# oneapi-src/ishmem

Hardware: AMD Instinct MI355X
Metric: GiB/s device-resident float32 sum-reduce at 1/2/4/8 PEs vs HBM+xGMI roofline (higher is better)
Workload: dtype f32

## Files before the change

include/ishmem_capi.h:

```cpp
#ifndef ISHMEM_AMD_CAPI_H
#define ISHMEM_AMD_CAPI_H

#include <stddef.h>
#include <stdint.h>

#ifdef __cplusplus
extern "C" {
#endif

typedef enum {
    ISHMEMI_OP_AND = 0,
    ISHMEMI_OP_OR = 1,
    ISHMEMI_OP_XOR = 2,
    ISHMEMI_OP_MAX = 3,
    ISHMEMI_OP_MIN = 4,
    ISHMEMI_OP_SUM = 5,
    ISHMEMI_OP_PROD = 6,
    ISHMEMI_OP_COUNT = 7
} ishmemi_c_op_t;

typedef enum {
    ISHMEMI_DT_INT8 = 0,
    ISHMEMI_DT_INT16 = 1,
    ISHMEMI_DT_INT32 = 2,
// ... 137 lines not shown
#define ISHMEMI_C_AMO_COUNT 14
int ishmemi_c_amo(int op, int dtype, void *dest, uint64_t value_bits, uint64_t cond_bits, int pe, uint64_t *fetched_bits);
int ishmemi_c_amo_nbi(int op, int dtype, void *fetch, void *dest, uint64_t value_bits, uint64_t cond_bits, int pe);

#define ISHMEMI_C_MAX_PES 16
#define ISHMEMI_C_MAX_TEAMS 64
#define ISHMEMI_C_DEV_PHASES 4
typedef struct {
    int32_t pe, npes;
    uint64_t timeout_ticks;
    char *heap_base;
    uint64_t heap_size;
    char *peer_heap[ISHMEMI_C_MAX_PES];
    uint32_t *my_dflags;
    uint32_t *peer_dflags[ISHMEMI_C_MAX_PES];
    uint32_t *epochs;
    uint32_t *err;
    int32_t team_start[ISHMEMI_C_MAX_TEAMS], team_stride[ISHMEMI_C_MAX_TEAMS];
    int32_t team_size[ISHMEMI_C_MAX_TEAMS], team_my_idx[ISHMEMI_C_MAX_TEAMS];
    uint64_t *dev_counts;
} ishmemi_c_device_ctx_t;
void *ishmemi_c_device_ctx(void);
int ishmemi_c_register_device_ctx_slot(const void *host_shadow);

const char *ishmemi_c_last_error(void);
int ishmemi_c_set_param(const char *name, long long value);
long long ishmemi_c_get_param(const char *name);
int ishmemi_c_phase_times(float *ms5);
int ishmemi_c_error_count(void);
size_t ishmemi_c_dtype_size(int dtype);
int ishmemi_c_op_dtype_valid(int op, int dtype);
int ishmemi_c_chunk_bounds(uint64_t nitems, int npes, int c, uint64_t *begin, uint64_t *end);
int ishmemi_c_path_limits(int npes, int colocated, long long *ll_limit, long long *fold_limit);
int ishmemi_c_bootstrap_selftest(int pe, int npes, const char *key, int value, int *out);
const char *ishmemi_c_version(void);

#ifdef __cplusplus
}
#endif

#endif
```

ishmem_amd/_lib.py:

```python
from __future__ import annotations

import ctypes
import os
from pathlib import Path

LIB_PATH = Path(__file__).resolve().parent / "libishmem_amd.so"
_VARIANT = os.environ.get("ISHMEM_AMD_LIB")

_vp, _i, _sz, _ll, _u64 = ctypes.c_void_p, ctypes.c_int, ctypes.c_size_t, ctypes.c_longlong, ctypes.c_uint64
PROTOTYPES = [
    ("ishmemi_c_init", _i, []),
    ("ishmemi_c_init_pe", _i, [_i, _i, _i, ctypes.c_char_p]),
    ("ishmemi_c_launch_info", _i, [ctypes.POINTER(_i), ctypes.POINTER(_i), ctypes.POINTER(_i), ctypes.c_char_p, _sz,
                                   ctypes.c_char_p, _sz]),
    ("ishmemi_c_finalize", _i, []),
    ("ishmemi_c_initialized", _i, []),
    ("ishmemi_c_my_pe", _i, []),
    ("ishmemi_c_n_pes", _i, []),
    ("ishmemi_c_device", _i, []),
    ("ishmemi_c_init_thread", _i, [_i, ctypes.POINTER(_i)]),
    ("ishmemi_c_query_thread", _i, [ctypes.POINTER(_i)]),
    ("ishmemi_c_malloc", _vp, [_sz]),
    ("ishmemi_c_align", _vp, [_sz, _sz]),
    ("ishmemi_c_calloc", _vp, [_sz, _sz]),
# ... 33 lines not shown
    ("ishmemi_c_get_on_stream", _i, [_vp, _vp, _sz, _i, _vp]),
    ("ishmemi_c_quiet", _i, []),
    ("ishmemi_c_fence", _i, []),
    ("ishmemi_c_quiet_on_stream", _i, [_vp]),
    ("ishmemi_c_read_all_u32", _i, [_vp, _vp, _sz, _i, _vp]),
    ("ishmemi_c_put_signal", _i, [_vp, _vp, _sz, _vp, _u64, _i, _i]),
    ("ishmemi_c_put_signal_nbi", _i, [_vp, _vp, _sz, _vp, _u64, _i, _i]),
    ("ishmemi_c_put_signal_on_stream", _i, [_vp, _vp, _sz, _vp, _u64, _i, _i, _vp]),
    ("ishmemi_c_signal_op", _i, [_vp, _u64, _i, _i]),
    ("ishmemi_c_signal_fetch", _i, [_vp, ctypes.POINTER(_u64)]),
    ("ishmemi_c_wait_until", _i, [_vp, _i, _i, _u64, ctypes.POINTER(_u64)]),
    ("ishmemi_c_test", _i, [_vp, _i, _i, _u64, ctypes.POINTER(_i)]),
    ("ishmemi_c_wait_until_on_stream", _i, [_vp, _i, _i, _u64, _vp, _vp, _vp]),
    ("ishmemi_c_amo", _i, [_i, _i, _vp, _u64, _u64, _i, ctypes.POINTER(_u64)]),
    ("ishmemi_c_amo_nbi", _i, [_i, _i, _vp, _vp, _u64, _u64, _i]),
    ("ishmemi_c_stream_wait_events", _i, [_vp, _vp, _sz]),
    ("ishmemi_c_stream_record_event", _i, [_vp, _vp]),
    ("ishmemi_c_collect", _i, [_i, _vp, _vp, _sz]),
    ("ishmemi_c_scan", _i, [_i, _i, _i, _vp, _vp, _sz]),
    ("ishmemi_c_scan_on_stream", _i, [_i, _i, _i, _vp, _vp, _sz, _vp, _vp]),
    ("ishmemi_c_broadcast", _i, [_i, _vp, _vp, _sz, _i]),
    ("ishmemi_c_broadcast_on_stream", _i, [_i, _vp, _vp, _sz, _i, _vp, _vp]),
    ("ishmemi_c_device_ctx", _vp, []),
    ("ishmemi_c_register_device_ctx_slot", _i, [_vp]),
    ("ishmemi_c_last_error", ctypes.c_char_p, []),
    ("ishmemi_c_set_param", _i, [ctypes.c_char_p, _ll]),
    ("ishmemi_c_get_param", _ll, [ctypes.c_char_p]),
    ("ishmemi_c_phase_times", _i, [ctypes.POINTER(ctypes.c_float)]),
    ("ishmemi_c_error_count", _i, []),
    ("ishmemi_c_dtype_size", _sz, [_i]),
    ("ishmemi_c_op_dtype_valid", _i, [_i, _i]),
    ("ishmemi_c_chunk_bounds", _i, [_u64, _i, _i, ctypes.POINTER(_u64), ctypes.POINTER(_u64)]),
    ("ishmemi_c_path_limits", _i, [_i, _i, ctypes.POINTER(_ll), ctypes.POINTER(_ll)]),
    ("ishmemi_c_bootstrap_selftest", _i, [_i, _i, ctypes.c_char_p, _i, ctypes.POINTER(_i)]),
    ("ishmemi_c_version", ctypes.c_char_p, []),
]

_lib = None


def load(build_if_missing: bool = True) -> ctypes.CDLL:
    global _lib
    if _lib is not None:
        return _lib
    if _VARIANT:
        lib = ctypes.CDLL(str(Path(_VARIANT).resolve()), mode=ctypes.RTLD_GLOBAL)
        for name, res, args in PROTOTYPES:
            fn = getattr(lib, name)
            fn.restype = res
            fn.argtypes = args
        _lib = lib
        return lib
    if build_if_missing:
        from . import _build
        if _build.needs_build():
            try:
                _build.build()
            except RuntimeError:
                if not LIB_PATH.exists():
                    raise
    if not LIB_PATH.exists():
        raise ImportError(f"ishmem_amd native library missing: {LIB_PATH} (run __graft_entry__.build())")
    lib = ctypes.CDLL(str(LIB_PATH), mode=ctypes.RTLD_GLOBAL)
    for name, res, args in PROTOTYPES:
        fn = getattr(lib, name)
        fn.restype = res
# ... 18 lines not shown
```

ishmem_amd/csrc/kernels.h:

```cpp
#pragma once
#include <hip/hip_runtime.h>
#include <stddef.h>
#include <stdint.h>

#include "types.h"

namespace ishmemi {

constexpr int kMaxPes = 16;
constexpr int kMaxBlocks = 1024;
constexpr int kPhases = 4;
constexpr int kPhaseStart = 0, kPhaseMid = 1, kPhaseEnd = 2, kPhaseSync = 3;
constexpr size_t kFlagWordsPerTeam = (size_t) kPhases * kMaxBlocks * kMaxPes;
constexpr size_t kTeamFlagBytes = kFlagWordsPerTeam * 4 + 256;
constexpr int kBlock = 256;
constexpr int kUnroll = 4;
constexpr int kFaninBlock = 64;
constexpr int kFaninMaxGrid = (int) ((1ull << 31) / kFaninBlock);

constexpr int kEpWords = 16;
constexpr int kLineWords = 16;
constexpr int kEpReplicas = 64;
constexpr int kEpRepLine = 1, kEpShardLine = kEpRepLine + kEpReplicas, kEpShards = 8;
constexpr int kEpTopLine = kEpShardLine + kEpShards;
// ... 109 lines not shown
constexpr int kRealignMaxGrid = (int) ((1ull << 31) / kRealignBlock);
#ifndef ISHMEMI_RS_REALIGN_BLOCK
#define ISHMEMI_RS_REALIGN_BLOCK 64
#endif
constexpr int kRsRealignBlock = ISHMEMI_RS_REALIGN_BLOCK;
#ifndef ISHMEMI_REALIGN_PEEL
#define ISHMEMI_REALIGN_PEEL 256
#endif
constexpr uint64_t kRealignPeel = ISHMEMI_REALIGN_PEEL;

struct FaninArgs {
    const char *src[kMaxFanin];
    char *dst;
    uint64_t head, nitems, tail;
    int nsrc;
    int realign;
    uint32_t shift[kMaxFanin];
    uint64_t total;
};

struct PhaseArgs {
    const char *src[kMaxPes];
    const char *dstp[kMaxPes];
    char *dst;
    uint64_t head, nitems, tail;
    uint64_t items_per_chunk;
    uint32_t elem;
    int p, me;
    int peer_nt;
    uint32_t shift;
    uint64_t total;
    int whole;
    int xcd_group;
};
hipError_t launch_rs_phase(int op, int dt, const PhaseArgs &a, hipStream_t s);
hipError_t launch_ag_phase(const PhaseArgs &a, hipStream_t s);

hipError_t launch_allreduce(int op, int dt, bool vec, const ReduceArgs &a, int grid,
                            hipStream_t s);
hipError_t launch_fanin(int op, int dt, bool vec, const FaninArgs &a, int grid, hipStream_t s);
hipError_t launch_team_sync(const ReduceArgs &a, hipStream_t s);
hipError_t launch_pull_probe(const FaninArgs &a, int policy, hipStream_t s);
void set_device_share(int share);
int device_share();
constexpr int kWaitSlotsDefault = 16;
void set_wait_slots(int slots);
int wait_slots();
void set_realign_grid_cap(int cap);
int realign_grid_cap();
void set_collect_realign(int on);
int collect_realign();
void set_phase_unaligned(int on);
int phase_unaligned();
hipError_t launch_occupy(int grid, uint64_t usec, hipStream_t s);
hipError_t launch_produce_u32(uint32_t *dst, const uint32_t *a, const uint32_t *b, uint64_t n, hipStream_t s);

struct RmaArgs {
    char *dst;
    const char *src;
    uint64_t head, nitems, tail;
};
hipError_t launch_rma_copy(const RmaArgs &a, bool put, int max_blocks, hipStream_t s);
hipError_t launch_read_all_u32(uint32_t *out, const uint32_t *p, uint64_t n, int grid, hipStream_t s);

constexpr int kSignalSet = 0, kSignalAdd = 1;
constexpr int kCmpEq = 1, kCmpLe = 6;
__host__ __device__ inline bool signal_compare(uint64_t v, int cmp, uint64_t c, int width, int is_signed)
{
    if (width == 4) {
        v = is_signed ? (uint64_t) (int64_t) (int32_t) (uint32_t) v : (uint64_t) (uint32_t) v;
        c = is_signed ? (uint64_t) (int64_t) (int32_t) (uint32_t) c : (uint64_t) (uint32_t) c;
    }
    const bool lt = is_signed ? (int64_t) v < (int64_t) c : v < c;
    switch (cmp) {
        case 1: return v == c;
        case 2: return v != c;
        case 3: return !lt && v != c;
        case 4: return !lt;
        case 5: return lt;
        case 6: return lt || v == c;
        default: return false;
    }
// ... 33 lines not shown
```

ishmem_amd/csrc/kernels.hip:

```cpp
#include "kernels_impl.h"

namespace ishmemi {

namespace {
int g_device_share = 1;
int g_wait_slots = kWaitSlotsDefault;
}
void set_device_share(int share) { g_device_share = share < 1 ? 1 : share; }
int device_share() { return g_device_share; }
void set_wait_slots(int slots) { g_wait_slots = slots < 1 ? 1 : slots; }
int wait_slots() { return g_wait_slots; }
int g_realign_grid_cap = 0;
void set_realign_grid_cap(int cap) { g_realign_grid_cap = cap < 0 ? 0 : cap; }
int realign_grid_cap() { return g_realign_grid_cap; }
int g_collect_realign = 1;
void set_collect_realign(int on) { g_collect_realign = on != 0; }
int collect_realign() { return g_collect_realign; }
int g_phase_unaligned = 1;
void set_phase_unaligned(int on) { g_phase_unaligned = on != 0; }
int phase_unaligned() { return g_phase_unaligned; }

#define ISHMEMI_DECL_OP(N)                                                                         \
    hipError_t launch_allreduce_op##N(int dt, bool vec, const ReduceArgs &a, int grid,             \
                                      hipStream_t s);                                              \
    hipError_t launch_fanin_op##N(int dt, bool vec, const FaninArgs &a, int grid, hipStream_t s); \
    hipError_t launch_ll_op##N(int dt, const LLArgs &a, hipStream_t s);                            \
    hipError_t launch_rs_phase_op##N(int dt, const PhaseArgs &a, hipStream_t s);
ISHMEMI_DECL_OP(0)
ISHMEMI_DECL_OP(1)
ISHMEMI_DECL_OP(2)
ISHMEMI_DECL_OP(3)
ISHMEMI_DECL_OP(4)
ISHMEMI_DECL_OP(5)
ISHMEMI_DECL_OP(6)

hipError_t launch_allreduce(int op, int dt, bool vec, const ReduceArgs &a, int grid, hipStream_t s)
{
    if (!op_dtype_valid(op, dt)) return hipErrorInvalidValue;
    switch (op) {
        case 0: return launch_allreduce_op0(dt, vec, a, grid, s);
        case 1: return launch_allreduce_op1(dt, vec, a, grid, s);
        case 2: return launch_allreduce_op2(dt, vec, a, grid, s);
        case 3: return launch_allreduce_op3(dt, vec, a, grid, s);
        case 4: return launch_allreduce_op4(dt, vec, a, grid, s);
        case 5: return launch_allreduce_op5(dt, vec, a, grid, s);
        case 6: return launch_allreduce_op6(dt, vec, a, grid, s);
        default: return hipErrorInvalidValue;
// ... 3 lines not shown
hipError_t launch_fanin(int op, int dt, bool vec, const FaninArgs &a, int grid, hipStream_t s)
{
    if (!op_dtype_valid(op, dt)) return hipErrorInvalidValue;
    switch (op) {
        case 0: return launch_fanin_op0(dt, vec, a, grid, s);
        case 1: return launch_fanin_op1(dt, vec, a, grid, s);
        case 2: return launch_fanin_op2(dt, vec, a, grid, s);
        case 3: return launch_fanin_op3(dt, vec, a, grid, s);
        case 4: return launch_fanin_op4(dt, vec, a, grid, s);
        case 5: return launch_fanin_op5(dt, vec, a, grid, s);
        case 6: return launch_fanin_op6(dt, vec, a, grid, s);
        default: return hipErrorInvalidValue;
    }
}

hipError_t launch_ll(int op, int dt, const LLArgs &a, hipStream_t s)
{
    if (!op_dtype_valid(op, dt)) return hipErrorInvalidValue;
    switch (op) {
        case 0: return launch_ll_op0(dt, a, s);
        case 1: return launch_ll_op1(dt, a, s);
        case 2: return launch_ll_op2(dt, a, s);
        case 3: return launch_ll_op3(dt, a, s);
        case 4: return launch_ll_op4(dt, a, s);
        case 5: return launch_ll_op5(dt, a, s);
        case 6: return launch_ll_op6(dt, a, s);
        default: return hipErrorInvalidValue;
    }
}

hipError_t launch_rs_phase(int op, int dt, const PhaseArgs &a, hipStream_t s)
{
    if (!op_dtype_valid(op, dt)) return hipErrorInvalidValue;
    switch (op) {
        case 0: return launch_rs_phase_op0(dt, a, s);
        case 1: return launch_rs_phase_op1(dt, a, s);
        case 2: return launch_rs_phase_op2(dt, a, s);
        case 3: return launch_rs_phase_op3(dt, a, s);
        case 4: return launch_rs_phase_op4(dt, a, s);
        case 5: return launch_rs_phase_op5(dt, a, s);
        case 6: return launch_rs_phase_op6(dt, a, s);
        default: return hipErrorInvalidValue;
    }
}

hipError_t launch_ag_phase(const PhaseArgs &a, hipStream_t s)
{
    const uint64_t blocks = (a.items_per_chunk + kFaninBlock - 1) / kFaninBlock;
    hipLaunchKernelGGL(ag_phase_kernel, dim3(phase_grid(ag_phase_kernel, (uint64_t) (a.p - 1) * blocks * kFaninBlock)),
                       dim3(kFaninBlock), 0, s, a);
    return hipGetLastError();
}

hipError_t launch_team_sync(const ReduceArgs &a, hipStream_t s)
{
    hipLaunchKernelGGL(team_sync_kernel, dim3(1), dim3(kBlock), 0, s, a);
    return hipGetLastError();
}

}
```

ishmem_amd/csrc/kernels_impl.h:

```cpp
#pragma once
#include <algorithm>
#include <map>
#include <mutex>
#include <type_traits>

#include "kernels.h"

namespace ishmemi {
namespace {

constexpr int kSysCoherent = 17;
constexpr int kNonTemporal = 2;
constexpr uint64_t kTile = (uint64_t) kBlock * kUnroll;
#ifndef ISHMEMI_AR_OCC
#define ISHMEMI_AR_OCC 4
#endif


template <typename T>
struct alignas(16) Vec {
    T e[16 / sizeof(T)];
};

template <typename T>
// ... 786 lines not shown
    if (i0 + tid < a.nitems) wt_store(make_rsrc(uniform_ptr(a.dst + wo)), tid * 16u, acc);
}

template <typename T, int OP, int NS>
__global__ __launch_bounds__(kRealignBlock) void fanin_realign_kernel(FaninArgs a)
{
    static_assert(NS == 1 || NS == 2, "realigned fan-in: 1 or 2 sources");
    __shared__ u32x4 edge[NS][kRealignWaves + 1];
    const uint32_t tid = threadIdx.x;
    const uint64_t stride = (uint64_t) gridDim.x * kRealignBlock;
    const uint64_t first = (uint64_t) blockIdx.x * kRealignBlock;
    if (stride >= a.nitems) {
        if (first < a.nitems) fanin_realign_block<T, OP, NS>(a, edge, first);
    } else {
        for (uint64_t i0 = first; i0 < a.nitems; i0 += stride) {
            fanin_realign_block<T, OP, NS>(a, edge, i0);
            __syncthreads();
        }
    }
    if (blockIdx.x == 0) {
        const uint64_t tail_off = a.head + a.nitems * (16 / sizeof(T));
        for (int pass = 0; pass < 2; ++pass) {
            const uint64_t cnt = pass == 0 ? a.head : a.tail;
            for (uint64_t t = tid; t < cnt; t += kRealignBlock) {
                const uint64_t e = pass == 0 ? t : tail_off + t;
                T acc = ((const T *) a.src[0])[e];
                if constexpr (NS == 2) acc = op1<T, OP>(acc, ((const T *) a.src[1])[e]);
                ((T *) a.dst)[e] = acc;
            }
        }
    }
}

template <typename T, int OP, int P, bool NT, int R>
__device__ __forceinline__ void rs_phase_item(const PhaseArgs &a, uint64_t wb, bool valid)
{
    using Item = Vec<T>;
    const uint32_t off = threadIdx.x * 16u;
    Item x[P];
#pragma unroll
    for (int k = 0; k < P; ++k) {
        const int j = (R + k) % P;
        if (!valid) continue;
        if (NT || j == a.me) x[k] = bload<Item>(make_rsrc(uniform_ptr(a.src[j] + wb)), off);
        else x[k] = cload<Item>(make_rsrc(uniform_ptr(a.src[j] + wb)), off);
    }
    Item acc = x[(P - R) % P];
#pragma unroll
    for (int j = 1; j < P; ++j) acc = op1<T, OP>(acc, x[(j - R + P) % P]);
    if (valid) wt_store(make_rsrc(uniform_ptr(a.dst + wb)), off, acc);
}

template <typename T, int OP, int P, bool NT, int R = 0>
__device__ __forceinline__ void rs_phase_dispatch(const PhaseArgs &a, int rot, uint64_t wb, bool valid)
{
    if constexpr (R == P - 1) {
        rs_phase_item<T, OP, P, NT, R>(a, wb, valid);
    } else {
        if (rot == R) rs_phase_item<T, OP, P, NT, R>(a, wb, valid);
        else rs_phase_dispatch<T, OP, P, NT, R + 1>(a, rot, wb, valid);
    }
}

template <typename T, int OP>
__device__ __forceinline__ void rs_phase_item_any(const PhaseArgs &a, uint64_t wb, bool valid)
{
    using Item = Vec<T>;
    if (!valid) return;
    const uint32_t off = threadIdx.x * 16u;
    Item acc;
    for (int j = 0; j < a.p; ++j) {
        Item x;
        if (j == a.me || a.peer_nt) x = nt_load((const Item *) (a.src[j] + wb + off));
        else x = cload<Item>(make_rsrc(uniform_ptr(a.src[j] + wb)), off);
        acc = j == 0 ? x : op1<T, OP>(acc, x);
    }
    wt_store(make_rsrc(uniform_ptr(a.dst + wb)), off, acc);
}

template <typename T, int OP>
__device__ __forceinline__ void rs_phase_edges(const PhaseArgs &a)
{
    const int p = a.p, me = a.me;
    if (blockIdx.x == 0) {
        const int tid = threadIdx.x;
        const uint64_t tail_off = a.head + a.nitems * (16 / sizeof(T));
        for (int region = 0; region < 2; ++region) {
            const bool owner = a.whole || (region == 0 ? me == 0 : me == p - 1);
            const uint64_t cnt = region == 0 ? a.head : a.tail;
            if (!owner || (uint64_t) tid >= cnt) continue;
            const uint64_t rbase = (region == 0 ? 0 : tail_off) * sizeof(T);
            const uint32_t off = (uint32_t) (tid * sizeof(T));
            T acc = T();
            for (int j = 0; j < p; ++j) {
                T x;
                if (j == me) x = ((const T *) (a.src[j] + rbase))[tid];
                else x = cload<T>(make_rsrc(uniform_ptr(a.src[j] + rbase)), off);
                acc = (j == 0) ? x : op1<T, OP>(acc, x);
            }
            wt_store(make_rsrc(uniform_ptr(a.dst + rbase)), off, acc);
        }
    }
}

__device__ __forceinline__ uint64_t xcd_grouped_block(uint64_t b, uint64_t grid)
{
    if (b >= (grid & ~63ull)) return b;
    return (b & ~63ull) | ((b & 7) << 3) | ((b >> 3) & 7);
}

template <typename T, int OP, int P>
__global__ __launch_bounds__(kFaninBlock) void rs_phase_kernel(PhaseArgs a)
{
    const int me = a.me;
    const uint64_t cs = a.whole ? 0 : min((uint64_t) me * a.items_per_chunk, a.nitems);
    const uint64_t ce = a.whole ? a.nitems : min(cs + a.items_per_chunk, a.nitems);
    const uint64_t head_bytes = a.head * sizeof(T);
    const uint64_t stride = (uint64_t) gridDim.x * kFaninBlock;
    const uint64_t blk = a.shift && a.xcd_group ? xcd_grouped_block(blockIdx.x, gridDim.x) : blockIdx.x;
    auto body = [&](auto nt) {
        for (uint64_t i0 = cs + blk * kFaninBlock; i0 < ce; i0 += stride) {
            const bool valid = i0 + threadIdx.x < ce;
            const uint64_t wb = head_bytes + i0 * 16;
            if constexpr (P > 0) rs_phase_dispatch<T, OP, P, decltype(nt)::value>(a, (int) ((i0 / kFaninBlock) % P), wb, valid);
            else rs_phase_item_any<T, OP>(a, wb, valid);
        }
    };
    if (a.peer_nt) {
        body(std::true_type{});
    } else {
        body(std::false_type{});
    }
    rs_phase_edges<T, OP>(a);
// ... 62 lines not shown
        const uint64_t je = min(js + a.items_per_chunk, a.nitems);
        const uint64_t i0 = js + (w / peers) * kFaninBlock;
        if (i0 + threadIdx.x < je) {
            const uint64_t wb = head_bytes + i0 * 16;
            const u32x4 x = a.peer_nt ? nt_load((const u32x4 *) (a.dstp[j] + wb + off))
                                      : cload<u32x4>(make_rsrc(uniform_ptr(a.dstp[j] + wb)), off);
            wt_store(make_rsrc(uniform_ptr(a.dst + wb)), off, x);
        }
    }
    if (blockIdx.x == 0) {
        const uint32_t tid = threadIdx.x;
        const uint64_t tail_b = (uint64_t) a.tail * a.elem;
        const uint64_t tail_base = head_bytes + a.nitems * 16;
        if (me != 0 && tid < head_bytes)
            a.dst[tid] = (char) cload<uint8_t>(make_rsrc(uniform_ptr(a.dstp[0])), tid);
        if (me != p - 1 && tid < tail_b)
            a.dst[tail_base + tid] = (char) cload<uint8_t>(make_rsrc(uniform_ptr(a.dstp[p - 1] + tail_base)), tid);
    }
}

template <typename K>
int phase_grid(K, uint64_t items)
{
    const uint64_t g = (items + kFaninBlock - 1) / kFaninBlock;
    return (int) std::max<uint64_t>(1, std::min<uint64_t>(g, (uint64_t) kFaninMaxGrid));
}

template <typename T, int OP>
hipError_t rs_phase_t(const PhaseArgs &a, hipStream_t s)
{
    const uint64_t cs = a.whole ? 0 : std::min((uint64_t) a.me * a.items_per_chunk, a.nitems);
    const uint64_t len = a.whole ? a.nitems : std::min(cs + a.items_per_chunk, a.nitems) - cs;
    auto go = [&](auto kernel) {
        hipLaunchKernelGGL(kernel, dim3(phase_grid(kernel, len)), dim3(kFaninBlock), 0, s, a);
    };
    if (a.shift && !phase_unaligned()) {
        uint64_t g = std::max<uint64_t>(1, std::min<uint64_t>((len + kRsRealignBlock - 1) / kRsRealignBlock,
                                                              (1ull << 31) / kRsRealignBlock));
        if (realign_grid_cap() > 0) g = std::min<uint64_t>(g, (uint64_t) realign_grid_cap());
        hipLaunchKernelGGL((rs_phase_realign_kernel<T, OP>), dim3((unsigned) g), dim3(kRsRealignBlock), 0, s, a);
    } else if (a.p == 2) go(rs_phase_kernel<T, OP, 2>);
    else if (a.p == 4) go(rs_phase_kernel<T, OP, 4>);
    else if (a.p == 8) go(rs_phase_kernel<T, OP, 8>);
    else go(rs_phase_kernel<T, OP, 0>);
    return hipGetLastError();
}

template <typename T, int OP>
__device__ __forceinline__ uint64_t fold8(uint64_t acc, uint64_t x)
{
    constexpr int K = 8 / sizeof(T);
    struct alignas(8) W {
        T e[K];
    };
    W a = __builtin_bit_cast(W, acc), b = __builtin_bit_cast(W, x);
#pragma unroll
    for (int i = 0; i < K; ++i) a.e[i] = op1<T, OP>(a.e[i], b.e[i]);
    return __builtin_bit_cast(uint64_t, a);
}

__device__ __forceinline__ uint64_t ll_load(const char *p, uint64_t valid)
{
    if (valid == 8) {
        if (((uintptr_t) p & 7) == 0) return *(const uint64_t *) p;
        if (((uintptr_t) p & 3) == 0)
            return (uint64_t) ((const uint32_t *) p)[0] | ((uint64_t) ((const uint32_t *) p)[1] << 32);
    }
// ... 230 lines not shown
```

ishmem_amd/csrc/runtime.cpp:

```cpp
#include <hip/hip_runtime.h>
#include <stdio.h>
#include <stdlib.h>
#include <string.h>
#include <strings.h>
#include <stdint.h>
#include <errno.h>
#include <sys/prctl.h>
#include <unistd.h>

#include <algorithm>
#include <chrono>
#include <limits>
#include <map>
#include <mutex>
#include <string>
#include <vector>

#include "bootstrap.h"
#include "kernels.h"
#include "types.h"

namespace ishmemi {
namespace {

// ... 134 lines not shown
    const char *b = s;
    while (*b == ' ' || *b == '\t') ++b;
    char *end = nullptr;
    errno = 0;
    const long long v = strtoll(b, &end, 10);
    const char *e = end;
    while (*e == ' ' || *e == '\t') ++e;
    if (end == b || *e || errno == ERANGE) {
        if (strncmp(name, "ISHMEM_", 7) == 0 && g_env_error.empty())
            g_env_error = std::string(name) + "='" + s + "' is not an integer";
        return dflt;
    }
    return v;
}

bool env_flag_false(const char *name)
{
    const char *s = getenv(name);
    return s && *s && (strcmp(s, "0") == 0 || strcasecmp(s, "false") == 0);
}
bool env_flag_true(const char *name)
{
    const char *s = getenv(name);
    return s && *s && !env_flag_false(name);
}

void warn_unknown_env()
{
    static const char *const known[] = {
        "DEBUG", "ENABLE_VERBOSE_PRINT", "STACK_PRINT_LIMIT", "ENABLE_GPU_IPC", "ENABLE_GPU_IPC_PIDFD",
        "SYMMETRIC_SIZE", "ENABLE_ACCESSIBLE_HOST_HEAP", "NBI_COUNT", "MWAIT_BURST", "SHMEM_LIB_NAME",
        "MPI_LIB_NAME", "PMI_LIB_NAME", "TEAMS_MAX", "TEAM_SHARED_ONLY_SELF", "RUNTIME", "RUNTIME_USE_OSHMPI", "ROOT",
        "PE", "NPES", "DEVICE", "BOOTSTRAP_KEY", "TIMEOUT_MS", "MAX_BLOCKS", "WAIT_SLOTS", "LL_MAX_BYTES",
        "ONESHOT_P2_MAX_BYTES", "PHASED_MIN_BYTES", "PHASED_PEER_NT", "STAGING_SIZE", "STAGING_SLOTS",
        "STAGED_COPY_KERNEL", "STREAM_ORDER", "FLAGS_KIND", "EP_UNCACHED", "BARRIER_KIND", "XGMI_LL_MAX_BYTES",
        "XGMI_FOLD_MAX_BYTES", "PUT_SIGNAL_FUSED_MAX_BYTES", "TEST_FLAGS_UNAVAILABLE", "TEST_PCI_BUS",
        "AMD_LIB", "OFFLOAD_ARCH", "BENCH_SAME_DEVICE", "BENCH_EMULATE_SHARE1", "BENCH_SETUP_WATCHDOG_S"};
    for (char **e = ::environ; e && *e; ++e) {
        if (strncmp(*e, "ISHMEM_", 7) != 0) continue;
        const char *name = *e + 7, *eq = strchr(name, '=');
        const size_t len = eq ? (size_t) (eq - name) : strlen(name);
        bool ok = false;
        for (const char *k : known) ok = ok || (strlen(k) == len && strncmp(k, name, len) == 0);
        if (!ok) fprintf(stderr, "[ishmem_amd] WARN: Environment variable 'ISHMEM_%.*s' is not a supported variable\n", (int) len, name);
    }
}

long long wait_slots_floor() { return std::max<long long>(1, env_ll("GPU_MAX_HW_QUEUES", 4)); }

struct Team {
    bool valid = false;
    int start = 0, stride = 1, size = 1;
    int my_idx = -1;
    int num_contexts = 0;
    bool colocated = true;
};

struct TeamMem {
    uint32_t *flags[kMaxPes] = {};
    uint64_t *ring[kMaxPes] = {};
    int pool_idx = -1;
    char *fold_scratch = nullptr;
    size_t fold_scratch_bytes = 0;
};

struct PoolBlock {
    uint32_t *ptr = nullptr;
    hipIpcMemHandle_t handle{};
    bool in_use = false;
};

constexpr long long kPhasedOff = std::numeric_limits<long long>::max();
constexpr long long kPhasedDefault = 4ll << 20;

struct PeRecord {
    int32_t pe, pid, device, flags_kind;
    int32_t flags_kind_requested;
    char pci_bus[32];
    uint64_t heap_size;
    int64_t max_blocks, ll_max_bytes, oneshot_p2, phased_min;
    uint64_t staging_bytes;
    int64_t staging_slots;
    int64_t xgmi_ll_max, xgmi_fold_max;
    hipIpcMemHandle_t heap_handle;
    hipIpcMemHandle_t flags_handle;
};

constexpr long long kPutSignalFusedDefault = 32 << 10;
constexpr int kWaitSlots = 16;
constexpr uint64_t kWaitSliceTicks = 100000;

struct State {
    std::mutex mu;
    bool initialized = false;
    int pe = 0, npes = 1, device = 0;
    ShmBootstrap boot;

    char *heap = nullptr;
    size_t heap_size = 0;
    std::map<size_t, size_t> free_list;
    std::map<size_t, size_t> used;
    char *peer_heap[kMaxPes] = {};

    uint32_t *flags = nullptr;
    int flags_kind = 0;
    uint32_t *peer_flags[kMaxPes] = {};
    int dev_id[kMaxPes] = {};
    TeamMem tmem[kMaxTeams];
    int teams_max = kTeamsMaxDefault;
    size_t team_block_bytes = 0;
    std::vector<PoolBlock> team_pool;
    std::map<std::pair<int, uint32_t>, void *> peer_pool;
    uint32_t *err_host = nullptr;
    uint32_t *err_dev = nullptr;
    uint64_t *exch_host = nullptr, *exch_dev = nullptr;
    uint32_t *done_host = nullptr, *done_dev = nullptr;
    uint32_t done_seq = 0;
    int block_spin = 2;
    ishmemi_c_device_ctx_t *dctx = nullptr;
    uint32_t *dev_epochs = nullptr;
    uint32_t *kern_ep = nullptr;

    char *team_scratch = nullptr;
    char *count_slots = nullptr;
    char *staging = nullptr;
    size_t staging_bytes = 0;
    hipStream_t copy_in = nullptr, copy_out = nullptr;
    hipStream_t rma_stream = nullptr;
    hipEvent_t rma_ev = nullptr;
    bool rma_pending = false;
    long long put_signal_fused_max = kPutSignalFusedDefault;
    hipStream_t wait_stream[kWaitSlots] = {};
    bool wait_busy[kWaitSlots] = {};
    char *wait_host = nullptr, *wait_dev = nullptr;
    hipStream_t last_stream = nullptr;
    bool last_stream_set = false;
    bool stream_order = false;
    long long oneshot_p2 = 32ll << 20;
    long long phased_min = kPhasedDefault;
    hipEvent_t order_ev = nullptr;
    hipEvent_t staging_ev = nullptr;
    bool staging_used = false;
    int staging_slots = kStagingSlotsDefault;
    int staged_copy_kernel = 0;
    bool test_flags_unavailable = false;
    int phased_peer_nt = 0;
    int ar_shifted = 1;
    int rs_xcd = 1;
    int direct_p2 = 1;
    int direct_max_pes = 4;
    int direct_inplace = 1;
    long long xgmi_ll_max = -1, xgmi_fold_max = -1;
    double xgmi_link_bps = 76.8e9;
    hipEvent_t ev_in[kMaxStagingSlots] = {}, ev_red[kMaxStagingSlots] = {}, ev_out[kMaxStagingSlots] = {};

    Team teams[kMaxTeams];
    int max_blocks = kMaxBlocks;
    long long ll_max_bytes = (long long) kLLDefaultBytes;
    long long timeout_ms = 60000;
    int debug = 0;
    int error_count = 0;
    uint64_t *trace = nullptr;
    bool phase_events = false, phase_recorded = false;
    hipEvent_t phase_ev[6] = {};
    double init_us[8] = {};
};

const char *const kInitPhase[8] = {"hip", "heap", "flags", "bootstrap", "ipc_heap", "ipc_flags", "teams", "total"};

State &S()
{
    static State s;
// ... 441 lines not shown
        scratch = m.fold_scratch + (d0 & 15);
    }
    const bool inplace_fold = scratch != nullptr;
    const bool direct = (fold_size && disjoint && (pl.vec || realign)) || inplace_fold;
    if ((pl.vec || realign) && (direct || (long long) nb >= s.phased_min)) {
        PhaseArgs ph;
        memset(&ph, 0, sizeof(ph));
        for (int j = 0; j < t.size; ++j) {
            ph.src[j] = a.src[j];
            ph.dstp[j] = a.dstp[j];
        }
        ph.dst = a.dst;
        ph.head = pl.head;
        ph.nitems = pl.nitems;
        ph.tail = pl.tail;
        ph.items_per_chunk = pl.items_per_chunk;
        ph.elem = (uint32_t) es;
        ph.p = t.size;
        ph.me = t.my_idx;
        ph.peer_nt = s.phased_peer_nt;
        ph.whole = direct ? 1 : 0;
        ph.xcd_group = s.rs_xcd && device_share() == 1 ? 1 : 0;
        if (inplace_fold) ph.dst = scratch;
        if (realign) {
            const uint64_t h = std::min<uint64_t>(n, ((16 - d0 % 16) % 16) / es);
            ph.head = h;
            ph.nitems = (n - h) * es / 16;
            ph.tail = n - h - ph.nitems * (16 / es);
            ph.items_per_chunk = items_per_chunk(ph.nitems, t.size);
            ph.shift = (uint32_t) ((s0 + h * es) % 16);
            ph.total = nb;
        }
        const bool ev = s.phase_events && !capturing(st);
        auto mark = [&](int k) -> int {
            if (ev) HIP_TRY(hipEventRecord(s.phase_ev[k], st));
            return 0;
        };
        if (mark(0)) return 1;
        if (team_barrier(s, team, a, st)) return 1;
        if (mark(1)) return 1;
        HIP_TRY(launch_rs_phase(op, dt, ph, st));
        if (mark(2)) return 1;
        if (!direct) {
            if (team_barrier(s, team, a, st)) return 1;
            if (mark(3)) return 1;
            HIP_TRY(launch_ag_phase(ph, st));
        } else if (mark(3)) {
            return 1;
        }
        if (mark(4)) return 1;
        if (team_barrier(s, team, a, st)) return 1;
        if (mark(5)) return 1;
        if (inplace_fold && launch_copy(dst, scratch, nb, st)) return 1;
        s.phase_recorded = s.phase_recorded || ev;
        return 0;
    }
    if (t.size == 2 && (long long) nb <= lim.oneshot && disjoint) {
        a.oneshot = 1;
        a.items_per_chunk = pl.nitems;
        a.seg_items = seg_items(pl.nitems);
        pl.grid = (int) std::max<uint64_t>(
            1, std::min<uint64_t>(nsegs(pl.nitems, a.seg_items), (uint64_t) s.max_blocks));
    }
    HIP_TRY(launch_allreduce(op, dt, pl.vec, a, pl.grid, st));
    return 0;
}

constexpr size_t kPinMinBytes = (size_t) 1 << 20;

bool pageable_host(const void *p)
{
    hipPointerAttribute_t attr;
    if (hipPointerGetAttributes(&attr, p) != hipSuccess) {
        (void) hipGetLastError();
        return true;
    }
// ... 1038 lines not shown
    if (env_flag_false("ISHMEM_ENABLE_GPU_IPC") && g_env_error.empty())
        g_env_error = std::string("ISHMEM_ENABLE_GPU_IPC=") + getenv("ISHMEM_ENABLE_GPU_IPC") +
                      " is not supported: ishmem_amd's collectives are IPC-only (peer loads over xGMI from "
                      "IPC-mapped heaps; there is no proxy path)";
    if (env_flag_true("ISHMEM_ENABLE_ACCESSIBLE_HOST_HEAP") && g_env_error.empty())
        g_env_error = std::string("ISHMEM_ENABLE_ACCESSIBLE_HOST_HEAP=") + getenv("ISHMEM_ENABLE_ACCESSIBLE_HOST_HEAP") +
                      " is not supported: the symmetric heap is device memory shared over IPC (host buffers "
                      "are accepted by every call and staged)";
    s.max_blocks = (int) std::min<long long>(kMaxBlocks, std::max<long long>(1, env_ll("ISHMEM_MAX_BLOCKS", kMaxBlocks)));
    s.timeout_ms = std::max<long long>(1, env_ll("ISHMEM_TIMEOUT_MS", 60000));
    s.ll_max_bytes = std::min<long long>((long long) kLLMaxBytes,
                                         std::max<long long>(0, env_bytes("ISHMEM_LL_MAX_BYTES", (long long) kLLDefaultBytes)));
    s.debug = debug_level();
    s.trace = nullptr;
    s.stream_order = env_ll("ISHMEM_STREAM_ORDER", 0) != 0;
    s.oneshot_p2 = std::max<long long>(0, env_bytes("ISHMEM_ONESHOT_P2_MAX_BYTES", 32ll << 20));
    s.phased_min = env_bytes("ISHMEM_PHASED_MIN_BYTES", kPhasedDefault);
    if (s.phased_min < 0) s.phased_min = kPhasedOff;
    s.staging_bytes = (env_size("ISHMEM_STAGING_SIZE", (size_t) 128 << 20) + kHeapAlign - 1) &
                      ~(size_t) (kHeapAlign - 1);
    s.staging_slots = (int) std::min<long long>(kMaxStagingSlots, std::max<long long>(2, env_ll("ISHMEM_STAGING_SLOTS", kStagingSlotsDefault)));
    s.staged_copy_kernel = (int) (env_ll("ISHMEM_STAGED_COPY_KERNEL", kStagedCopyKernelDefault) & 3);
    const size_t heap_request = env_size("ISHMEM_SYMMETRIC_SIZE", (size_t) 4 << 30);
    const int first_kind = (int) std::min<long long>(kFlagsCoarse, std::max<long long>(0, env_ll("ISHMEM_FLAGS_KIND", 0)));
#ifdef ISHMEMI_TEST_HOOKS
    s.test_flags_unavailable = env_ll("ISHMEM_TEST_FLAGS_UNAVAILABLE", 0) != 0;
#else
    for (const char *hook : {"ISHMEM_TEST_FLAGS_UNAVAILABLE", "ISHMEM_TEST_PCI_BUS"})
        if (getenv(hook) && g_env_error.empty())
            g_env_error = std::string(hook) + " is a test hook, honoured only by libishmem_amd_testhooks.so";
#endif
    const bool ep_uncached = env_ll("ISHMEM_EP_UNCACHED", 0) != 0;
    s.phased_peer_nt = env_ll("ISHMEM_PHASED_PEER_NT", 0) != 0;
    s.teams_max = kTeamsMaxDefault;
    if (const char *tm = getenv("ISHMEM_TEAMS_MAX"); tm && *tm) {
        const long long v = env_ll("ISHMEM_TEAMS_MAX", kTeamsMaxDefault);
        if (v < 0 && g_env_error.empty())
            g_env_error = std::string("ISHMEM_TEAMS_MAX='") + tm + "' is not a team count";
        else if (v > kMaxTeams && g_env_error.empty())
            g_env_error = "ISHMEM_TEAMS_MAX=" + std::to_string(v) + ": requested " + std::to_string(v) +
                          " teams, but only " + std::to_string(kMaxTeams) + " are supported";
        s.teams_max = (int) std::min<long long>(kMaxTeams, std::max<long long>(kPredefTeams, v));
    }
    s.xgmi_ll_max = std::max<long long>(-1, env_bytes("ISHMEM_XGMI_LL_MAX_BYTES", -1));
    s.xgmi_fold_max = std::max<long long>(-1, env_bytes("ISHMEM_XGMI_FOLD_MAX_BYTES", -1));
    s.xgmi_link_bps = 76.8e9;
    s.put_signal_fused_max = std::max<long long>(0, env_bytes("ISHMEM_PUT_SIGNAL_FUSED_MAX_BYTES", kPutSignalFusedDefault));
    if (const char *bk = getenv("ISHMEM_BARRIER_KIND"); bk && *bk && strcasecmp(bk, "kernel") != 0 && g_env_error.empty())
        g_env_error = std::string("ISHMEM_BARRIER_KIND='") + bk +
                      "' is not supported: team barriers are the one-workgroup barrier kernel ('kernel')";
    if (!g_env_error.empty()) {
        const std::string e = g_env_error;
        g_env_error.clear();
        return fail("init: " + e);
    }
    warn_unknown_env();

    using clk = std::chrono::steady_clock;
    const auto t_start = clk::now();
    auto t_mark = t_start;
    auto phase_done = [&](int k) {
        const auto now = clk::now();
        s.init_us[k] = std::chrono::duration<double, std::micro>(now - t_mark).count();
        t_mark = now;
        if (s.debug > 1) {
            fprintf(stderr, "[ishmem_amd] PE %d init: %s done (%.1f ms)\n", pe, kInitPhase[k], s.init_us[k] / 1000.0);
// ... 37 lines not shown

    for (int i = 0; i < kMaxPes; ++i) {
        s.peer_heap[i] = nullptr;
        s.peer_flags[i] = nullptr;
    }
    s.peer_heap[pe] = s.heap;
    s.peer_flags[pe] = s.flags;
    for (int i = 0; i < kMaxPes; ++i) s.dev_id[i] = 0;
    phase_done(2);

    if (npes > 1) {
        struct PtracerWindow {
            PtracerWindow() { prctl(PR_SET_PTRACER, PR_SET_PTRACER_ANY, 0, 0, 0); }
            ~PtracerWindow() { prctl(PR_SET_PTRACER, 0, 0, 0, 0); }
        } ptracer_window;
        std::string err;
        if (s.boot.attach(pe, npes, key, (int) std::max<long long>(s.timeout_ms, 10000), err))
            return fail(err);
        PeRecord mine{};
        mine.pe = pe;
        mine.pid = (int32_t) getpid();
        mine.device = s.device;
        mine.flags_kind = s.flags_kind;
        mine.flags_kind_requested = first_kind;
        mine.heap_size = s.heap_size;
        mine.max_blocks = s.max_blocks;
        mine.ll_max_bytes = s.ll_max_bytes;
        mine.oneshot_p2 = s.oneshot_p2;
        mine.phased_min = s.phased_min;
        mine.staging_bytes = s.staging_bytes;
        mine.staging_slots = s.staging_slots;
        mine.xgmi_ll_max = s.xgmi_ll_max;
        mine.xgmi_fold_max = s.xgmi_fold_max;
        if (hipDeviceGetPCIBusId(mine.pci_bus, sizeof(mine.pci_bus), s.device) != hipSuccess) {
            (void) hipGetLastError();
            snprintf(mine.pci_bus, sizeof(mine.pci_bus), "dev%d", s.device);
        }
#ifdef ISHMEMI_TEST_HOOKS
        if (const char *fake = getenv("ISHMEM_TEST_PCI_BUS"))
            snprintf(mine.pci_bus, sizeof(mine.pci_bus), "%s", fake);
#endif
        if (hipError_t e = hipIpcGetMemHandle(&mine.heap_handle, s.heap); e != hipSuccess)
            return fail(std::string("init: hipIpcGetMemHandle of the symmetric heap: ") + hipGetErrorString(e) + ipc_hint());
        mine.flags_handle = flags_handle;
        PeRecord all[kMaxPes];
        if (s.boot.allgather(&mine, all, sizeof(PeRecord), err)) return fail(err);
        phase_done(3);
        for (int j = 0; j < npes; ++j) {
            s.ll_max_bytes = std::min<long long>(s.ll_max_bytes, all[j].ll_max_bytes);
            s.oneshot_p2 = std::min<long long>(s.oneshot_p2, all[j].oneshot_p2);
            s.phased_min = std::max<long long>(s.phased_min, all[j].phased_min);
            s.staging_bytes = std::min<size_t>(s.staging_bytes, all[j].staging_bytes);
            s.staging_slots = (int) std::min<int64_t>(s.staging_slots, all[j].staging_slots);
            if (all[j].xgmi_ll_max >= 0)
                s.xgmi_ll_max = s.xgmi_ll_max < 0 ? all[j].xgmi_ll_max : std::min<long long>(s.xgmi_ll_max, all[j].xgmi_ll_max);
            if (all[j].xgmi_fold_max >= 0)
                s.xgmi_fold_max = s.xgmi_fold_max < 0 ? all[j].xgmi_fold_max
                                                       : std::min<long long>(s.xgmi_fold_max, all[j].xgmi_fold_max);
        }
        int share = 0;
        for (int j = 0; j < npes; ++j)
            share += strncmp(all[j].pci_bus, mine.pci_bus, sizeof(mine.pci_bus)) == 0;
        for (int j = 0; j < npes; ++j) {
            s.dev_id[j] = j;
            for (int k = 0; k < j; ++k)
                if (strncmp(all[j].pci_bus, all[k].pci_bus, sizeof(all[j].pci_bus)) == 0) {
                    s.dev_id[j] = s.dev_id[k];
                    break;
                }
        }
        bool coarse_forced = false;
        for (int j = 0; j < npes; ++j) coarse_forced = coarse_forced || all[j].flags_kind_requested == kFlagsCoarse;
        set_device_share(share);
        for (int j = 0; j < npes; ++j) {
            if (j == pe) continue;
            if (all[j].heap_size != s.heap_size)
                return fail("init: ISHMEM_SYMMETRIC_SIZE differs between PEs");
            if (all[j].device != s.device) {
                int can = 0;
                if (hipDeviceCanAccessPeer(&can, s.device, all[j].device) != hipSuccess || !can)
// ... 1277 lines not shown
const char *ishmemi_c_last_error(void) { return g_last_error.c_str(); }

int ishmemi_c_phase_times(float *ms5)
{
    State &s = S();
    if (!ms5) return fail("phase_times: null output");
    if (!s.phase_recorded || !s.phase_ev[0]) return fail("phase_times: no phased reduce recorded (set_param phase_events 1)");
    HIP_TRY(hipEventSynchronize(s.phase_ev[5]));
    for (int k = 0; k < 5; ++k) HIP_TRY(hipEventElapsedTime(&ms5[k], s.phase_ev[k], s.phase_ev[k + 1]));
    return 0;
}

int ishmemi_c_set_param(const char *name, long long value)
{
    State &s = S();
    std::lock_guard<std::mutex> lk(s.mu);
    const std::string n = name ? name : "";
    if (n == "max_blocks") s.max_blocks = (int) std::min<long long>(kMaxBlocks, std::max<long long>(1, value));
    else if (n == "staged_copy_kernel") s.staged_copy_kernel = (int) (value & 3);
    else if (n == "wait_slots") {
        if (value < wait_slots_floor())
            return fail("set_param: wait_slots " + std::to_string(value) + " is below " +
                        std::to_string(wait_slots_floor()) + " (GPU_MAX_HW_QUEUES), see ISHMEM_WAIT_SLOTS");
        set_wait_slots((int) std::min<long long>(1 << 20, value));
    }
    else if (n == "timeout_ms") s.timeout_ms = std::max<long long>(1, value);
    else if (n == "stream_order") s.stream_order = value != 0;
    else if (n == "oneshot_p2_max_bytes") s.oneshot_p2 = std::max<long long>(0, value);
    else if (n == "phased_min_bytes") s.phased_min = value < 0 ? kPhasedOff : value;
    else if (n == "ll_max_bytes") s.ll_max_bytes = std::min<long long>((long long) kLLMaxBytes, std::max<long long>(0, value));
    else if (n == "put_signal_fused_max_bytes") s.put_signal_fused_max = std::max<long long>(0, value);
    else if (n == "debug") s.debug = (int) value;
    else if (n == "phased_peer_nt") s.phased_peer_nt = value != 0;
    else if (n == "xgmi_ll_max_bytes") s.xgmi_ll_max = std::max<long long>(-1, value);
    else if (n == "xgmi_fold_max_bytes") s.xgmi_fold_max = std::max<long long>(-1, value);
    else if (n == "xgmi_link_mbps") {
        if (value <= 0) return fail("set_param: xgmi_link_mbps must be positive");
        s.xgmi_link_bps = (double) value * 1e6;
    }
    else if (n == "realign_grid_cap") set_realign_grid_cap((int) std::min<long long>(std::max<long long>(value, 0), 1 << 30));
    else if (n == "collect_realign") set_collect_realign((int) (value != 0));
    else if (n == "ar_shifted") s.ar_shifted = value != 0;
    else if (n == "rs_xcd") s.rs_xcd = value != 0;
    else if (n == "direct_p2") s.direct_p2 = value != 0;
    else if (n == "direct_inplace") s.direct_inplace = value != 0;
    else if (n == "block_spin") s.block_spin = (int) std::min<long long>(std::max<long long>(value, 0), 2);
    else if (n == "direct_max_pes") s.direct_max_pes = (int) std::min<long long>(std::max<long long>(value, 2), kMaxPes);
    else if (n == "phase_unaligned") set_phase_unaligned((int) (value != 0));
    else if (n == "trace_buffer") s.trace = (uint64_t *) (uintptr_t) value;
    else if (n == "phase_events") {
        if (value && !s.phase_ev[0])
            for (hipEvent_t &e : s.phase_ev) HIP_TRY(hipEventCreate(&e));
        s.phase_events = value != 0;
    }
    else return fail("set_param: unknown parameter " + n);
    return 0;
}

long long ishmemi_c_get_param(const char *name)
{
    State &s = S();
    const std::string n = name ? name : "";
    if (n == "max_blocks") return s.max_blocks;
    if (n == "staged_copy_kernel") return s.staged_copy_kernel;
    if (n == "wait_slots") return wait_slots();
    if (n == "timeout_ms") return s.timeout_ms;
    if (n == "stream_order") return s.stream_order ? 1 : 0;
    if (n == "oneshot_p2_max_bytes") return s.oneshot_p2;
    if (n == "phased_min_bytes") return s.phased_min == kPhasedOff ? -1 : s.phased_min;
    if (n == "ll_max_bytes") return s.ll_max_bytes;
    if (n == "put_signal_fused_max_bytes") return s.put_signal_fused_max;
    if (n == "ll_capacity_bytes") return (long long) ll_capacity(s.npes);
    if (n == "ll_limit_bytes") return team_limits(s, s.teams[0]).ll;
    if (n == "fold_limit_bytes") return team_limits(s, s.teams[0]).fold;
    if (n == "team_colocated") return s.teams[0].colocated ? 1 : 0;
    if (n == "xgmi_ll_max_bytes") return s.xgmi_ll_max;
    if (n == "xgmi_fold_max_bytes") return s.xgmi_fold_max;
    if (n == "xgmi_link_mbps") return (long long) (s.xgmi_link_bps / 1e6);
    if (n == "teams_max") return s.teams_max;
    if (n == "flag_block_bytes") return s.initialized ? (long long) (kBaseAllocBytes + s.team_block_bytes) : 0;
    if (n == "flag_block_pool_bytes") return (long long) (s.team_pool.size() * kTeamAllocBytes);
    if (n == "flag_block_bytes_round5") return (long long) kRound5FlagBytes;
    for (int k = 0; k < 8; ++k)
        if (n == std::string("init_us_") + kInitPhase[k]) return (long long) s.init_us[k];
    if (n == "debug") return s.debug;
    if (n == "phased_peer_nt") return s.phased_peer_nt;
    if (n == "realign_grid_cap") return realign_grid_cap();
    if (n == "collect_realign") return collect_realign();
    if (n == "ar_shifted") return s.ar_shifted;
    if (n == "rs_xcd") return s.rs_xcd;
    if (n == "direct_p2") return s.direct_p2;
    if (n == "direct_inplace") return s.direct_inplace;
    if (n == "block_spin") return s.block_spin;
    if (n == "direct_max_pes") return s.direct_max_pes;
    if (n == "phase_unaligned") return phase_unaligned();
    if (n == "flags_fine_grained") return s.flags_kind != kFlagsCoarse ? 1 : 0;
    if (n == "flags_kind") return s.flags_kind;
    if (n == "staging_bytes") return (long long) s.staging_bytes;
    if (n == "staging_slots") return s.staging_slots;
    if (n == "heap_bytes") return (long long) s.heap_size;
    if (n == "device_share") return device_share();
    if (n == "launch_words") return (long long) (uintptr_t) s.kern_ep;
    if (n == "cu_count") {
        int dev = 0, cus = 0;
        if (hipGetDevice(&dev) != hipSuccess ||
            hipDeviceGetAttribute(&cus, hipDeviceAttributeMultiprocessorCount, dev) != hipSuccess) {
            (void) hipGetLastError();
            return -1;
        }
        return cus;
    }
    return -1;
}

int ishmemi_c_error_count(void)
{
    State &s = S();
    int pending = 0;
    if (s.err_host)
        for (int t = 0; t <= kMaxTeams; ++t)
            pending += __atomic_load_n(&s.err_host[t], __ATOMIC_ACQUIRE) != 0;
    return s.error_count + pending;
}

size_t ishmemi_c_dtype_size(int dtype)
{
    return (dtype >= 0 && dtype < ISHMEMI_DT_COUNT) ? dtype_size(dtype) : 0;
}

int ishmemi_c_op_dtype_valid(int op, int dtype) { return op_dtype_valid(op, dtype) ? 1 : 0; }

int ishmemi_c_chunk_bounds(uint64_t nitems, int npes, int c, uint64_t *begin, uint64_t *end)
{
    if (npes < 1 || c < 0 || c >= npes || !begin || !end) return 1;
    const uint64_t ipc = npes > 1 ? items_per_chunk(nitems, npes) : nitems;
    *begin = std::min<uint64_t>((uint64_t) c * ipc, nitems);
    *end = std::min<uint64_t>(*begin + ipc, nitems);
    return 0;
}

int ishmemi_c_path_limits(int npes, int colocated, long long *ll_limit, long long *fold_limit)
{
    if (npes < 1 || npes > kMaxPes || !ll_limit || !fold_limit) return fail("path_limits: invalid arguments");
    State &s = S();
    std::lock_guard<std::mutex> lk(s.mu);
    const PathLimits r = path_limits(s, npes, colocated != 0);
    *ll_limit = r.ll;
    *fold_limit = r.fold;
    return 0;
}

int ishmemi_c_bootstrap_selftest(int pe, int npes, const char *key, int value, int *out)
{
    ShmBootstrap b;
    std::string err;
    if (b.attach(pe, npes, key ? key : "selftest", 20000, err)) return fail(err);
    if (b.allgather(&value, out, sizeof(int), err)) return fail(err);
    if (b.barrier(err)) return fail(err);
    return 0;
}

const char *ishmemi_c_version(void) { return "ishmem_amd 0.1.0 (reduction path; ref ishmem 1.5.1)"; }

}
```

Baseline: 3148.

## Push reduced chunks to all peers, skipping barrier and allgather phase

Adds a push mode to the phased reduce-scatter kernel. Each PE writes its reduced chunk directly into every peer's destination buffer instead of only its own. When push is active (on by default for colocated teams), the separate team barrier and allgather phase launch are skipped, which removes one kernel launch and one synchronization per reduce. The PE-wide setting is agreed at init via allgather. An optional phase grid cap knob is also added. The risk is heavier remote write traffic from the reduce kernel over xGMI, and peers reading results must still be ordered by some later sync.

```diff
diff --git a/include/ishmem_capi.h b/include/ishmem_capi.h
--- a/include/ishmem_capi.h
+++ b/include/ishmem_capi.h
@@ -193,6 +193,7 @@
 int ishmemi_c_op_dtype_valid(int op, int dtype);
 int ishmemi_c_chunk_bounds(uint64_t nitems, int npes, int c, uint64_t *begin, uint64_t *end);
 int ishmemi_c_path_limits(int npes, int colocated, long long *ll_limit, long long *fold_limit);
+long long ishmemi_c_agree_push_reduce(const long long *values, int n);
 int ishmemi_c_bootstrap_selftest(int pe, int npes, const char *key, int value, int *out);
 const char *ishmemi_c_version(void);
 
diff --git a/ishmem_amd/_lib.py b/ishmem_amd/_lib.py
--- a/ishmem_amd/_lib.py
+++ b/ishmem_amd/_lib.py
@@ -89,6 +89,7 @@
     ("ishmemi_c_op_dtype_valid", _i, [_i, _i]),
     ("ishmemi_c_chunk_bounds", _i, [_u64, _i, _i, ctypes.POINTER(_u64), ctypes.POINTER(_u64)]),
     ("ishmemi_c_path_limits", _i, [_i, _i, ctypes.POINTER(_ll), ctypes.POINTER(_ll)]),
+    ("ishmemi_c_agree_push_reduce", _ll, [ctypes.POINTER(_ll), _i]),
     ("ishmemi_c_bootstrap_selftest", _i, [_i, _i, ctypes.c_char_p, _i, ctypes.POINTER(_i)]),
     ("ishmemi_c_version", ctypes.c_char_p, []),
 ]
diff --git a/ishmem_amd/csrc/kernels.h b/ishmem_amd/csrc/kernels.h
--- a/ishmem_amd/csrc/kernels.h
+++ b/ishmem_amd/csrc/kernels.h
@@ -165,6 +165,7 @@
     uint64_t total;
     int whole;
     int xcd_group;
+    int push;
 };
 hipError_t launch_rs_phase(int op, int dt, const PhaseArgs &a, hipStream_t s);
 hipError_t launch_ag_phase(const PhaseArgs &a, hipStream_t s);
@@ -181,6 +182,8 @@
 int wait_slots();
 void set_realign_grid_cap(int cap);
 int realign_grid_cap();
+void set_phase_grid_cap(int cap);
+int phase_grid_cap();
 void set_collect_realign(int on);
 int collect_realign();
 void set_phase_unaligned(int on);
diff --git a/ishmem_amd/csrc/kernels.hip b/ishmem_amd/csrc/kernels.hip
--- a/ishmem_amd/csrc/kernels.hip
+++ b/ishmem_amd/csrc/kernels.hip
@@ -13,6 +13,9 @@
 int g_realign_grid_cap = 0;
 void set_realign_grid_cap(int cap) { g_realign_grid_cap = cap < 0 ? 0 : cap; }
 int realign_grid_cap() { return g_realign_grid_cap; }
+int g_phase_grid_cap = 0;
+void set_phase_grid_cap(int cap) { g_phase_grid_cap = cap < 0 ? 0 : cap; }
+int phase_grid_cap() { return g_phase_grid_cap; }
 int g_collect_realign = 1;
 void set_collect_realign(int on) { g_collect_realign = on != 0; }
 int collect_realign() { return g_collect_realign; }
@@ -82,6 +85,7 @@
 hipError_t launch_rs_phase(int op, int dt, const PhaseArgs &a, hipStream_t s)
 {
     if (!op_dtype_valid(op, dt)) return hipErrorInvalidValue;
+    if (a.push && (a.whole || (a.shift && !phase_unaligned()))) return hipErrorInvalidValue;
     switch (op) {
         case 0: return launch_rs_phase_op0(dt, a, s);
         case 1: return launch_rs_phase_op1(dt, a, s);
diff --git a/ishmem_amd/csrc/kernels_impl.h b/ishmem_amd/csrc/kernels_impl.h
--- a/ishmem_amd/csrc/kernels_impl.h
+++ b/ishmem_amd/csrc/kernels_impl.h
@@ -842,6 +842,22 @@
     }
 }
 
+template <int P, typename I>
+__device__ __forceinline__ void push_store(const PhaseArgs &a, uint64_t wb, uint32_t off, const I &v)
+{
+    wt_store(make_rsrc(uniform_ptr(a.dst + wb)), off, v);
+    if constexpr (P > 0) {
+#pragma unroll
+        for (int k = 1; k < P; ++k)
+            wt_store(make_rsrc(uniform_ptr(a.dstp[(a.me + k) % P] + wb)), off, v);
+    } else {
+        for (int k = 1; k < a.p; ++k) {
+            const int j = a.me + k < a.p ? a.me + k : a.me + k - a.p;
+            wt_store(make_rsrc(uniform_ptr(a.dstp[j] + wb)), off, v);
+        }
+    }
+}
+
 template <typename T, int OP, int P, bool NT, int R>
 __device__ __forceinline__ void rs_phase_item(const PhaseArgs &a, uint64_t wb, bool valid)
 {
@@ -858,7 +874,9 @@
     Item acc = x[(P - R) % P];
 #pragma unroll
     for (int j = 1; j < P; ++j) acc = op1<T, OP>(acc, x[(j - R + P) % P]);
-    if (valid) wt_store(make_rsrc(uniform_ptr(a.dst + wb)), off, acc);
+    if (!valid) return;
+    if (a.push) push_store<P>(a, wb, off, acc);
+    else wt_store(make_rsrc(uniform_ptr(a.dst + wb)), off, acc);
 }
 
 template <typename T, int OP, int P, bool NT, int R = 0>
@@ -885,7 +903,8 @@
         else x = cload<Item>(make_rsrc(uniform_ptr(a.src[j] + wb)), off);
         acc = j == 0 ? x : op1<T, OP>(acc, x);
     }
-    wt_store(make_rsrc(uniform_ptr(a.dst + wb)), off, acc);
+    if (a.push) push_store<0>(a, wb, off, acc);
+    else wt_store(make_rsrc(uniform_ptr(a.dst + wb)), off, acc);
 }
 
 template <typename T, int OP>
@@ -908,7 +927,8 @@
                 else x = cload<T>(make_rsrc(uniform_ptr(a.src[j] + rbase)), off);
                 acc = (j == 0) ? x : op1<T, OP>(acc, x);
             }
-            wt_store(make_rsrc(uniform_ptr(a.dst + rbase)), off, acc);
+            if (a.push) push_store<0>(a, rbase, off, acc);
+            else wt_store(make_rsrc(uniform_ptr(a.dst + rbase)), off, acc);
         }
     }
 }
@@ -1037,7 +1057,9 @@
     const uint64_t cs = a.whole ? 0 : std::min((uint64_t) a.me * a.items_per_chunk, a.nitems);
     const uint64_t len = a.whole ? a.nitems : std::min(cs + a.items_per_chunk, a.nitems) - cs;
     auto go = [&](auto kernel) {
-        hipLaunchKernelGGL(kernel, dim3(phase_grid(kernel, len)), dim3(kFaninBlock), 0, s, a);
+        int g = phase_grid(kernel, len);
+        if (phase_grid_cap() > 0) g = std::min(g, phase_grid_cap());
+        hipLaunchKernelGGL(kernel, dim3(g), dim3(kFaninBlock), 0, s, a);
     };
     if (a.shift && !phase_unaligned()) {
         uint64_t g = std::max<uint64_t>(1, std::min<uint64_t>((len + kRsRealignBlock - 1) / kRsRealignBlock,
diff --git a/ishmem_amd/csrc/runtime.cpp b/ishmem_amd/csrc/runtime.cpp
--- a/ishmem_amd/csrc/runtime.cpp
+++ b/ishmem_amd/csrc/runtime.cpp
@@ -190,7 +190,7 @@
         "SYMMETRIC_SIZE", "ENABLE_ACCESSIBLE_HOST_HEAP", "NBI_COUNT", "MWAIT_BURST", "SHMEM_LIB_NAME",
         "MPI_LIB_NAME", "PMI_LIB_NAME", "TEAMS_MAX", "TEAM_SHARED_ONLY_SELF", "RUNTIME", "RUNTIME_USE_OSHMPI", "ROOT",
         "PE", "NPES", "DEVICE", "BOOTSTRAP_KEY", "TIMEOUT_MS", "MAX_BLOCKS", "WAIT_SLOTS", "LL_MAX_BYTES",
-        "ONESHOT_P2_MAX_BYTES", "PHASED_MIN_BYTES", "PHASED_PEER_NT", "STAGING_SIZE", "STAGING_SLOTS",
+        "ONESHOT_P2_MAX_BYTES", "PHASED_MIN_BYTES", "PHASED_PEER_NT", "PUSH_REDUCE", "STAGING_SIZE", "STAGING_SLOTS",
         "STAGED_COPY_KERNEL", "STREAM_ORDER", "FLAGS_KIND", "EP_UNCACHED", "BARRIER_KIND", "XGMI_LL_MAX_BYTES",
         "XGMI_FOLD_MAX_BYTES", "PUT_SIGNAL_FUSED_MAX_BYTES", "TEST_FLAGS_UNAVAILABLE", "TEST_PCI_BUS",
         "AMD_LIB", "OFFLOAD_ARCH", "BENCH_SAME_DEVICE", "BENCH_EMULATE_SHARE1", "BENCH_SETUP_WATCHDOG_S"};
@@ -230,6 +230,8 @@
 
 constexpr long long kPhasedOff = std::numeric_limits<long long>::max();
 constexpr long long kPhasedDefault = 4ll << 20;
+constexpr int kPushReduceDefault = 1, kPushReduceMax = 2;
+int clamp_push_reduce(long long v) { return (int) std::min<long long>(kPushReduceMax, std::max<long long>(0, v)); }
 
 struct PeRecord {
     int32_t pe, pid, device, flags_kind;
@@ -240,6 +242,7 @@
     uint64_t staging_bytes;
     int64_t staging_slots;
     int64_t xgmi_ll_max, xgmi_fold_max;
+    int64_t push_reduce;
     hipIpcMemHandle_t heap_handle;
     hipIpcMemHandle_t flags_handle;
 };
@@ -296,6 +299,8 @@
     bool stream_order = false;
     long long oneshot_p2 = 32ll << 20;
     long long phased_min = kPhasedDefault;
+    int push_reduce = kPushReduceDefault;
+    long long phased_push_calls = 0, phased_pull_calls = 0;
     hipEvent_t order_ev = nullptr;
     hipEvent_t staging_ev = nullptr;
     bool staging_used = false;
@@ -803,6 +808,11 @@
             ph.total = nb;
         }
         const bool ev = s.phase_events && !capturing(st);
+        const bool push = !direct && (disjoint || d0 == s0) && !s.phase_events &&
+                          (s.push_reduce >= 2 || (s.push_reduce == 1 && t.colocated)) &&
+                          !(ph.shift && !phase_unaligned());
+        ph.push = push ? 1 : 0;
+        if (!direct) ++(push ? s.phased_push_calls : s.phased_pull_calls);
         auto mark = [&](int k) -> int {
             if (ev) HIP_TRY(hipEventRecord(s.phase_ev[k], st));
             return 0;
@@ -812,7 +822,7 @@
         if (mark(1)) return 1;
         HIP_TRY(launch_rs_phase(op, dt, ph, st));
         if (mark(2)) return 1;
-        if (!direct) {
+        if (!direct && !push) {
             if (team_barrier(s, team, a, st)) return 1;
             if (mark(3)) return 1;
             HIP_TRY(launch_ag_phase(ph, st));
@@ -1917,6 +1927,8 @@
 #endif
     const bool ep_uncached = env_ll("ISHMEM_EP_UNCACHED", 0) != 0;
     s.phased_peer_nt = env_ll("ISHMEM_PHASED_PEER_NT", 0) != 0;
+    s.push_reduce = clamp_push_reduce(env_ll("ISHMEM_PUSH_REDUCE", kPushReduceDefault));
+    s.phased_push_calls = s.phased_pull_calls = 0;
     s.teams_max = kTeamsMaxDefault;
     if (const char *tm = getenv("ISHMEM_TEAMS_MAX"); tm && *tm) {
         const long long v = env_ll("ISHMEM_TEAMS_MAX", kTeamsMaxDefault);
@@ -2020,6 +2032,7 @@
         mine.staging_slots = s.staging_slots;
         mine.xgmi_ll_max = s.xgmi_ll_max;
         mine.xgmi_fold_max = s.xgmi_fold_max;
+        mine.push_reduce = s.push_reduce;
         if (hipDeviceGetPCIBusId(mine.pci_bus, sizeof(mine.pci_bus), s.device) != hipSuccess) {
             (void) hipGetLastError();
             snprintf(mine.pci_bus, sizeof(mine.pci_bus), "dev%d", s.device);
@@ -2034,6 +2047,11 @@
         PeRecord all[kMaxPes];
         if (s.boot.allgather(&mine, all, sizeof(PeRecord), err)) return fail(err);
         phase_done(3);
+        {
+            long long pr[kMaxPes];
+            for (int j = 0; j < npes; ++j) pr[j] = all[j].push_reduce;
+            s.push_reduce = (int) ishmemi_c_agree_push_reduce(pr, npes);
+        }
         for (int j = 0; j < npes; ++j) {
             s.ll_max_bytes = std::min<long long>(s.ll_max_bytes, all[j].ll_max_bytes);
             s.oneshot_p2 = std::min<long long>(s.oneshot_p2, all[j].oneshot_p2);
@@ -3377,6 +3395,11 @@
     else if (n == "put_signal_fused_max_bytes") s.put_signal_fused_max = std::max<long long>(0, value);
     else if (n == "debug") s.debug = (int) value;
     else if (n == "phased_peer_nt") s.phased_peer_nt = value != 0;
+    else if (n == "push_reduce") {
+        if (value < 0 || value > kPushReduceMax) return fail("set_param: push_reduce must be 0, 1 or 2");
+        s.push_reduce = (int) value;
+    }
+    else if (n == "phase_grid_cap") set_phase_grid_cap((int) std::min<long long>(std::max<long long>(value, 0), 1 << 30));
     else if (n == "xgmi_ll_max_bytes") s.xgmi_ll_max = std::max<long long>(-1, value);
     else if (n == "xgmi_fold_max_bytes") s.xgmi_fold_max = std::max<long long>(-1, value);
     else if (n == "xgmi_link_mbps") {
@@ -3430,6 +3453,10 @@
         if (n == std::string("init_us_") + kInitPhase[k]) return (long long) s.init_us[k];
     if (n == "debug") return s.debug;
     if (n == "phased_peer_nt") return s.phased_peer_nt;
+    if (n == "push_reduce") return s.push_reduce;
+    if (n == "phased_push_calls") return s.phased_push_calls;
+    if (n == "phased_pull_calls") return s.phased_pull_calls;
+    if (n == "phase_grid_cap") return phase_grid_cap();
     if (n == "realign_grid_cap") return realign_grid_cap();
     if (n == "collect_realign") return collect_realign();
     if (n == "ar_shifted") return s.ar_shifted;
@@ -3495,6 +3522,13 @@
     return 0;
 }
 
+long long ishmemi_c_agree_push_reduce(const long long *values, int n)
+{
+    long long r = kPushReduceMax;
+    for (int j = 0; values && j < n; ++j) r = std::min<long long>(r, clamp_push_reduce(values[j]));
+    return n > 0 && values ? r : kPushReduceDefault;
+}
+
 int ishmemi_c_bootstrap_selftest(int pe, int npes, const char *key, int value, int *out)
 {
     ShmBootstrap b;
```

New measurement: 3147. Within noise of the previous version (-0.0%).
